# archinetai/audio-diffusion-pytorch

Measured on AMD Instinct MI355X. Metric: denoising steps/s (UNetV0 fwd+bwd) at [B,2,2**18], higher is better.
Workload: dtype f32; 1 GPU; BASELINE.json configs[1]: unconditional DiffusionModel(UNetV0 channels=[8,32,64,128,256,512,512,1024,1024], factors=[1,4,4,4,2,2,2,2,2], items=[1,2,2,2,2,2,2,4,4]) fwd+bwd, audio=randn(4,2,2**18) per GPU, random-init weights; per_gpu_batch=4, global_batch=4, length=262144, launch=hipGraph replay, parallelism=single, collective_world_size=1, collectives_in_graph=False, optimizer=none (the metric is fwd+bwd; gradients for all 176M parameters are produced)

## Files before the change

### audio_diffusion_pytorch_amd/_C.py

```python
import ctypes
import os
from ctypes import POINTER, Structure, c_float, c_int, c_int64, c_void_p

import torch

_PKG_DIR = os.path.dirname(os.path.abspath(__file__))
LIB_PATH = os.path.join(_PKG_DIR, "libadp_hip.so")

_lib = None
_allow_cpu = False

ERRORS = {-1: "bad shape", -2: "unsupported configuration", -3: "misaligned pointer", -4: "kernel launch failed",
          -5: "null pointer"}

P = c_void_p
I = c_int64
F = c_float


class ConvDesc(Structure):
    _fields_ = [(n, c_void_p) for n in ("x", "x2", "w", "bias", "pro_stats", "pro_gamma", "pro_beta", "e_scale",
                                        "res", "out", "out_pre")] + \
               [(n, c_int64) for n in ("B", "R", "R1", "Lin", "M", "N", "KT", "stride", "dil", "pad", "up",
                                       "transposed", "prologue", "groups", "store", "sp", "e_bstride")] + \
# ... 99 lines not shown
    "adp_arv_step": (c_int, [P, P, P, I, I, I, I, P, P, P]),
    "adp_arv_plane": (c_int, [P, I, I, I, P, P]),
}

ABI["adp_lt.h"] = {
    "adp_lt_conv_out_len": (I, [I, I, I, I]),
    "adp_lt_convt_out_len": (I, [I, I, I, I]),
    "adp_lt_conv": (c_int, [P, P, I, I, I, I, I, I, I, I, P, P]),
    "adp_lt_convt": (c_int, [P, P, I, I, I, I, I, I, I, I, I, P, P]),
    "adp_lt_wgrad_ws_bytes": (I, [I, I, I, I, I]),
    "adp_lt_wgrad": (c_int, [P, P, I, I, I, I, I, I, I, I, I, P, P, P]),
}

ABI["adp_enc.h"] = {
    "adp_enc_down_out_len": (I, [I, I]),
    "adp_enc_down_fwd": (c_int, [P, P, P, I, I, I, I, I, P, P]),
    "adp_enc_down_dgrad": (c_int, [P, P, I, I, I, I, I, P, P]),
    "adp_enc_down_wgrad_ws_bytes": (I, [I, I, I, I, I]),
    "adp_enc_down_wgrad": (c_int, [P, P, I, I, I, I, I, P, P, P, P]),
    "adp_enc_tanh_fwd": (c_int, [P, I, P, P]),
    "adp_enc_tanh_bwd": (c_int, [P, P, I, P, P]),
}

ABI["adp_t5.h"] = {
    "adp_t5_embed": (c_int, [P, P, I, I, I, P, P]),
    "adp_t5_rmsnorm": (c_int, [P, P, I, I, F, P, P]),
    "adp_t5_linear_ws_bytes": (I, [I, I, I]),
    "adp_t5_linear": (c_int, [P, P, P, I, I, I, I, P, P, P]),
    "adp_t5_attn": (c_int, [P, P, P, P, I, I, I, I, I, P, P]),
}

ABI["adp_rng.h"] = {
    "adp_philox_bits": (c_int, [P, I, P, P]),
    "adp_randn": (c_int, [P, I, P, P]),
    "adp_v_inpaint_step_rng": (c_int, [P, P, P, P, P, P, I, P, P]),
}

ABI["adp_clip.h"] = {
    "adp_clip_ws_bytes": (I, [I, I]),
    "adp_clip_scale": (c_int, [P, P, P, I, I, I, F, F, P, P, P]),
    "adp_clip_apply": (c_int, [P, P, I, I, P, P]),
    "adp_clip_step": (c_int, [P, P, P, P, P, I, P, I, I, P, P, P, P]),
}

ABI["adp_gated.h"] = {
    "adp_gated_linear_ws_bytes": (I, [I, I, I]),
    "adp_gated_linear": (c_int, [P, P, P, I, I, I, I, P, P, P]),
}

ABI["adp_sde.h"] = {
    "adp_v_step_eta": (c_int, [P, P, P, P, I, P, I, I, P, P]),
}

ABI["adp_rf.h"] = {
    "adp_rf_noise": (c_int, [P, P, P, I, I, P, P, P]),
    "adp_rf_step": (c_int, [P, P, P, P, I, I, P, I, I, P, P, P]),
}

ABI["adp_edm.h"] = {
    "adp_edm_noise": (c_int, [P, P, P, F, I, I, P, P, P]),
    "adp_edm_step": (c_int, [P, P, P, P, P, I, I, P, I, I, P, P, P]),
}

ABI["adp_repaint.h"] = {
    "adp_repaint_v_step": (c_int, [P, P, P, P, P, P, I, P, I, I, P, P]),
    "adp_repaint_rf_step": (c_int, [P, P, P, P, P, P, I, P, I, I, P, P]),
    "adp_repaint_k_step": (c_int, [P, P, P, P, P, P, I, P, I, I, P, P]),
}

ABI["adp_spec.h"] = {
    "adp_spec_loss_ws_bytes": (I, [I, I, I, I, P, P, I]),
    "adp_spec_loss_fwd": (c_int, [P, P, I, I, I, I, P, P, P, P, F, F, F, F, F, F, P, P, P]),
    "adp_spec_loss_bwd": (c_int, [P, P, P, P, I, I, I, I, P, P, P, P, P, F, F, F, F, F, F, P, P, P]),
    "adp_spec_fir": (c_int, [P, P, I, I, I, P, P]),
}

ABI["adp_distill.h"] = {
    "adp_distill_comb": (c_int, [P, P, P, P, I, I, I, P, P]),
    "adp_distill_wmse_ws_bytes": (I, [I, I]),
    "adp_distill_wmse_fwd": (c_int, [P, P, P, I, I, P, P, P]),
    "adp_distill_wmse_bwd": (c_int, [P, P, P, P, I, I, P, P]),
}


HEADER_SOURCE = {"adp_ar.h": "elementwise.hip", "adp_lt.h": "lt.hip", "adp_enc.h": "encoder.hip", "adp_t5.h": "t5.hip",
                 "adp_rng.h": "rng.hip", "adp_clip.h": "clip.hip", "adp_gated.h": "gated.hip", "adp_sde.h": "sde.hip",
                 "adp_rf.h": "rf.hip", "adp_edm.h": "edm.hip", "adp_repaint.h": "repaint.hip", "adp_spec.h": "spectral.hip",
                 "adp_distill.h": "distill.hip"}

SIGNATURES = {}
for _header, _table in ABI.items():
    for _name in _table:
        if _name in SIGNATURES:
            _first = next(h for h, t in ABI.items() if _name in t)
            raise ImportError(f"{_name} is in the tables of both {_first} and {_header}: one header declares an entry point")
    SIGNATURES.update(_table)


def _bind(path: str):
    lib = ctypes.CDLL(path)
    for name, (res, args) in SIGNATURES.items():
        fn = getattr(lib, name)
        fn.restype = res
        fn.argtypes = args
    return lib


def lib():
    global _lib
    if _lib is None:
        if not os.path.exists(LIB_PATH):
            raise RuntimeError(
                f"{LIB_PATH} is missing: build the gfx950 kernels first "
                "(python -m audio_diffusion_pytorch_amd.build or __graft_entry__.build()); "
                "audio_diffusion_pytorch_amd has no CPU/PyTorch fallback path")
        _lib = _bind(LIB_PATH)
    return _lib


def _testing_use_library(path, allow_cpu: bool):
    global _lib, _allow_cpu
    _lib = _bind(path) if path is not None else None
    _allow_cpu = allow_cpu


def stream() -> int:
    if _allow_cpu and not torch.cuda.is_available():
        return 0
    return torch.cuda.current_stream().cuda_stream


def ptr(t, dtype=torch.float32):
    if t is None:
        return None
    if t.dtype != dtype:
        raise TypeError(f"adp kernel argument must be {dtype}; got {t.dtype}")
    if not t.is_contiguous():
        raise ValueError("adp kernels need contiguous tensors")
    if not t.is_cuda and not _allow_cpu:
        raise RuntimeError("adp kernels run on MI355X (HIP) tensors only; got a CPU tensor and there is no CPU path")
    return t.data_ptr()


def check(code: int, what: str):
    if code != 0:
        raise RuntimeError(f"{what} failed: {ERRORS.get(code, code)} ({code})")


PROFILE = None
_TAG = None
REPLAY = None


def tag(**meta):
    global _TAG
    if PROFILE is not None:
        _TAG = meta


def _decode_trace(text: str) -> str:
    import re
    names = []
    for item in text.split("\n"):
        if not item:
            continue
        kern, _, site = item.partition("@")
        kern = kern.strip()
        while kern.startswith("(") and kern.endswith(")"):
            kern = kern[1:-1].strip()
        m = re.search(r"\[(?:with )?([^\]]*)\]\s*$", site)
        env = {}
# ... 60 lines not shown
```

### audio_diffusion_pytorch_amd/csrc/linear.hip

```cpp
#include "adp_rt.h"
#include "adp.h"
#include "conv_internal.h"

namespace {

constexpr int LIN_BMAX = 16;
constexpr int LIN_KC = 1024;
constexpr int LIN_RPW = 8;
static inline int64_t lin_rpw(int64_t N) { return N >= 4096 ? LIN_RPW : 1; }

__device__ __forceinline__ float lin_act(float x, int act) {
  return act == 1 ? adp_silu(x) : (act == 2 ? adp_gelu(x) : x);
}

__device__ __forceinline__ void lin_stage(const float* x, int64_t B, int64_t K, int64_t k0, int kc, int act,
                                          float* xs) {
  for (int e = threadIdx.x; e < (int)B * LIN_KC; e += 256) {
    const int b = e / LIN_KC, k = e - b * LIN_KC;
    xs[e] = (k < kc) ? lin_act(x[b * K + k0 + k], act) : 0.0f;
  }
}

template <int BT>
__global__ __launch_bounds__(256) void linear_fwd_kernel(const float* x, const float* w, const float* bias,
                                                         int64_t B, int64_t K, int64_t N, int act, int post,
                                                         int64_t ybstride, float* y, int rpw) {
  __shared__ float xs[BT * LIN_KC];
  const int lane = threadIdx.x & 63, wave = threadIdx.x >> 6;
  const int64_t nbase = ((int64_t)blockIdx.x * 4 + wave) * rpw;
  const bool vec = (K % 4 == 0);
  for (int64_t k0 = 0; k0 < K; k0 += LIN_KC) {
    const int kc = (int)((K - k0) < LIN_KC ? (K - k0) : LIN_KC);
    __syncthreads();
    lin_stage(x, B, K, k0, kc, act, xs);
    __syncthreads();
    for (int r = 0; r < rpw; ++r) {
      const int64_t n = nbase + r;
      if (n >= N) break;
      float acc[BT];
#pragma unroll
      for (int b = 0; b < BT; ++b) acc[b] = 0.0f;
      const float* wr = w + n * K + k0;
#pragma unroll 4
      for (int k = lane * 4; k < kc; k += 256) {
        float w0, w1, w2, w3;
        if (vec) {
          const float4 wv = *reinterpret_cast<const float4*>(wr + k);
          w0 = wv.x; w1 = wv.y; w2 = wv.z; w3 = wv.w;
        } else {
          w0 = wr[k];
          w1 = (k + 1 < kc) ? wr[k + 1] : 0.0f;
          w2 = (k + 2 < kc) ? wr[k + 2] : 0.0f;
          w3 = (k + 3 < kc) ? wr[k + 3] : 0.0f;
        }
#pragma unroll
        for (int b = 0; b < BT; ++b) {
          if (b < B) {
            const float* xr = xs + b * LIN_KC + k;
            acc[b] = fmaf(w0, xr[0], fmaf(w1, xr[1], fmaf(w2, xr[2], fmaf(w3, xr[3], acc[b]))));
          }
        }
      }
#pragma unroll
      for (int b = 0; b < BT; ++b) {
        const float sres = adp_wave_sum(acc[b]);
        if (lane == 0 && b < B) {
          float v = sres + ((k0 == 0 && bias) ? bias[n] : 0.0f);
          if (k0 > 0) v += y[b * ybstride + n];
          if (post == 2 && k0 + LIN_KC >= K) v = adp_gelu(v);
          y[b * ybstride + n] = v;
        }
      }
    }
  }
}

constexpr int LIN_NR = 64;

template <int BT>
__global__ __launch_bounds__(256) void linear_bwd_data_kernel(const float* dy, int64_t dybstride, const float* w,
                                                              int64_t B, int64_t K, int64_t N, float* ws) {
  constexpr int NR = LIN_NR, RPW = NR / 4;
  __shared__ float dys[BT * NR];
  __shared__ __attribute__((aligned(16))) float part[3][BT][256];
// ... 38 lines not shown
    }
  }
  if (wave > 0) {
#pragma unroll
    for (int b = 0; b < BT; ++b)
#pragma unroll
      for (int q = 0; q < 4; ++q) part[wave - 1][b][lane * 4 + q] = acc[b][q];
  }
  __syncthreads();
  if (wave == 0 && k < K) {
#pragma unroll
    for (int b = 0; b < BT; ++b) {
      if (b < B) {
        float* o = ws + ((int64_t)blockIdx.x * B + b) * K + k;
#pragma unroll
        for (int q = 0; q < 4; ++q) {
          const float v = ((acc[b][q] + part[0][b][lane * 4 + q]) + part[1][b][lane * 4 + q]) + part[2][b][lane * 4 + q];
          if (k + q < K) o[q] = v;
        }
      }
    }
  }
}

template <int BT>
__global__ __launch_bounds__(256) void linear_bwd_weight_kernel(const float* dy, int64_t dybstride, const float* x,
                                                                int64_t B, int64_t K, int64_t N, int act,
                                                                int accumulate, float* dw, float* dbias, int rpw) {
  __shared__ __attribute__((aligned(16))) float xs[BT * LIN_KC];
  const int lane = threadIdx.x & 63, wave = threadIdx.x >> 6;
  const int64_t nbase = ((int64_t)blockIdx.x * 4 + wave) * rpw;
  const bool vec = (K % 4 == 0) && ((reinterpret_cast<uintptr_t>(dw) & 15) == 0);
  float dfirst[BT];
#pragma unroll
  for (int b = 0; b < BT; ++b) dfirst[b] = (b < B && nbase < N) ? dy[b * dybstride + nbase] : 0.0f;
  for (int64_t k0 = 0; k0 < K; k0 += LIN_KC) {
    const int kc = (int)((K - k0) < LIN_KC ? (K - k0) : LIN_KC);
    __syncthreads();
    lin_stage(x, B, K, k0, kc, act, xs);
    __syncthreads();
    for (int r = 0; r < rpw; ++r) {
      const int64_t n = nbase + r;
      if (n >= N) break;
      float d[BT];
#pragma unroll
      for (int b = 0; b < BT; ++b) d[b] = r == 0 ? dfirst[b] : ((b < B) ? dy[b * dybstride + n] : 0.0f);
      if (k0 == 0 && dbias && lane == 0) {
        float s = 0.0f;
#pragma unroll
        for (int b = 0; b < BT; ++b) s += d[b];
        dbias[n] = accumulate ? dbias[n] + s : s;
      }
      float* orow = dw + n * K + k0;
      if (vec) {
        for (int k = lane * 4; k < kc; k += 256) {
          f32x4 sv = {0.0f, 0.0f, 0.0f, 0.0f};
#pragma unroll
          for (int b = 0; b < BT; ++b)
            if (b < B) {
              const f32x4 xv = *reinterpret_cast<const f32x4*>(xs + b * LIN_KC + k);
#pragma unroll
              for (int j = 0; j < 4; ++j) sv[j] = fmaf(d[b], xv[j], sv[j]);
            }
          if (accumulate) {
            const f32x4 o = *reinterpret_cast<const f32x4*>(orow + k);
#pragma unroll
            for (int j = 0; j < 4; ++j) sv[j] += o[j];
          }
          *reinterpret_cast<f32x4*>(orow + k) = sv;
        }
      } else {
        for (int k = lane; k < kc; k += 64) {
          float s = 0.0f;
#pragma unroll
          for (int b = 0; b < BT; ++b)
            if (b < B) s = fmaf(d[b], xs[b * LIN_KC + k], s);
          orow[k] = accumulate ? orow[k] + s : s;
        }
      }
    }
  }
}

}

#define LIN_DISPATCH(B, CALL)                   \
  do {                                          \
    if ((B) <= 4) { constexpr int BT = 4; CALL; }        \
    else if ((B) <= 8) { constexpr int BT = 8; CALL; }   \
    else { constexpr int BT = 16; CALL; }       \
  } while (0)

extern "C" int adp_linear_fwd(const float* x, const float* w, const float* bias, int64_t B, int64_t K, int64_t N,
                              int64_t act, int64_t post, float* y, int64_t y_bstride, void* stream) {
  if (!x || !w || !y) return ADP_ERR_NULL;
  if (B <= 0 || B > LIN_BMAX || K <= 0 || N <= 0) return ADP_ERR_SHAPE;
  if (act < 0 || act > 2 || (post != 0 && post != 2)) return ADP_ERR_UNSUPPORTED;
  if (y_bstride == 0) y_bstride = N;
  const int64_t rpw = lin_rpw(N);
  dim3 grid((unsigned)adp_cdiv(N, 4 * rpw));
  LIN_DISPATCH(B, ADP_LAUNCH((linear_fwd_kernel<BT>), grid, dim3(256), stream, x, w, bias, B, K, N, (int)act,
                             (int)post, y_bstride, y, (int)rpw));
  return ADP_LAUNCH_OK();
}

extern "C" int64_t adp_linear_bwd_data_ws_bytes(int64_t B, int64_t K, int64_t N) {
  if (B <= 0 || K <= 0 || N <= 0) return ADP_ERR_SHAPE;
  return adp_cdiv(N, LIN_NR) * B * K * (int64_t)sizeof(float);
}

extern "C" int adp_linear_bwd_data(const float* dy, int64_t dy_bstride, const float* w, int64_t B, int64_t K,
                                   int64_t N, int64_t accumulate, float* dxa, float* ws, void* stream) {
  if (!dy || !w || !dxa || !ws) return ADP_ERR_NULL;
  if (B <= 0 || B > LIN_BMAX || K <= 0 || N <= 0) return ADP_ERR_SHAPE;
  if (dy_bstride == 0) dy_bstride = N;
  const int64_t P = adp_cdiv(N, LIN_NR);
  if (P > 2147483647 || adp_cdiv(K, 256) > 65535) return ADP_ERR_SHAPE;
  LIN_DISPATCH(B, ADP_LAUNCH((linear_bwd_data_kernel<BT>), dim3((unsigned)P, (unsigned)adp_cdiv(K, 256)), dim3(256),
                             stream, dy, dy_bstride, w, B, K, N, ws));
  return adp_wgrad_reduce(ws, P, B * K, 0, dxa, nullptr, (int)accumulate, stream);
}

extern "C" int adp_linear_bwd_weight(const float* dy, int64_t dy_bstride, const float* x, int64_t B, int64_t K,
                                     int64_t N, int64_t act, int64_t accumulate, float* dw, float* dbias,
                                     void* stream) {
  if (!dy || !x || !dw) return ADP_ERR_NULL;
  if (B <= 0 || B > LIN_BMAX || K <= 0 || N <= 0) return ADP_ERR_SHAPE;
  if (act < 0 || act > 2) return ADP_ERR_UNSUPPORTED;
  if (dy_bstride == 0) dy_bstride = N;
  const int64_t rpw = lin_rpw(N);
  dim3 grid((unsigned)adp_cdiv(N, 4 * rpw));
  LIN_DISPATCH(B, ADP_LAUNCH((linear_bwd_weight_kernel<BT>), grid, dim3(256), stream, dy, dy_bstride, x, B, K, N,
                             (int)act, (int)accumulate, dw, dbias, (int)rpw));
  return ADP_LAUNCH_OK();
}
```

### audio_diffusion_pytorch_amd/ops.py

```python
import contextlib
import ctypes
import math
import os
from ctypes import byref
from typing import Optional, Tuple

import torch
from torch import Tensor

from . import _C
from ._C import ConvDesc, WgradDesc, ptr

GN_EPS = 1e-5
MODULATION_LN_EPS = 1e-5
ATTENTION_LN_EPS = 1e-5


def _ws(nbytes: int, like: Tensor) -> Tensor:
    return torch.empty(max(1, (nbytes + 3) // 4), dtype=torch.float32, device=like.device)


def conv_out_len(Lin: int, KT: int, stride: int, dil: int, pad: int, up: int) -> int:
    return (Lin * up + 2 * pad - dil * (KT - 1) - 1) // stride + 1

# ... 377 lines not shown
    return dx, dgb


LIN_ROWS = 16


def linear_fwd(x: Tensor, w: Tensor, bias: Optional[Tensor], act: int = 0, post: int = 0,
               y: Optional[Tensor] = None) -> Tensor:
    B, K = x.shape
    N = w.shape[0]
    if y is None:
        y = torch.empty((B, N), dtype=torch.float32, device=x.device)
    _C.tag(bytes=4 * (w.numel() + x.numel() + y.numel()), shape=f"B{B} K{K} N{N}")
    for b0 in range(0, B, LIN_ROWS):
        nb = min(LIN_ROWS, B - b0)
        _C.call("adp_linear_fwd", ptr(x[b0:b0 + nb]), ptr(w), ptr(bias), nb, K, N, act, post, ptr(y[b0:b0 + nb]), N,
                _C.stream())
    return y


def linear_bwd_data(dy: Tensor, w: Tensor, dxa: Optional[Tensor] = None, accumulate: bool = False) -> Tensor:
    B, N = dy.shape
    K = w.shape[1]
    if dxa is None:
        dxa = torch.empty((B, K), dtype=torch.float32, device=dy.device)
    ws = _ws(_C.query("adp_linear_bwd_data_ws_bytes", min(B, LIN_ROWS), K, N), dy)
    _C.tag(bytes=4 * (w.numel() + B * N + dxa.numel()), shape=f"B{B} K{K} N{N}")
    for b0 in range(0, B, LIN_ROWS):
        nb = min(LIN_ROWS, B - b0)
        _C.call("adp_linear_bwd_data", ptr(dy[b0:b0 + nb]), N, ptr(w), nb, K, N, int(accumulate),
                ptr(dxa[b0:b0 + nb]), ptr(ws), _C.stream())
    return dxa


def linear_bwd_weight(dy: Tensor, x: Tensor, act: int = 0, dw: Optional[Tensor] = None,
                      dbias: Optional[Tensor] = None, want_bias: bool = True, accumulate: bool = False,
                      rows: Optional[int] = None, dy_bstride: Optional[int] = None):
    if rows is None:
        B, N = dy.shape
        dy_bstride = N
        dy = dy.reshape(-1)
    else:
        B, N = x.shape[0], rows
    K = x.shape[1]
    if dw is None:
        dw = torch.empty((N, K), dtype=torch.float32, device=dy.device)
    if dbias is None and want_bias:
        dbias = torch.empty((N,), dtype=torch.float32, device=dy.device)
    _C.tag(bytes=4 * (dw.numel() + B * N + x.numel()), shape=f"B{B} K{K} N{N}")
    for b0 in range(0, B, LIN_ROWS):
        nb = min(LIN_ROWS, B - b0)
        _C.call("adp_linear_bwd_weight", ptr(dy[b0 * dy_bstride:]), dy_bstride, ptr(x[b0:b0 + nb]), nb, K, N, act,
                int(accumulate or b0 > 0), ptr(dw), ptr(dbias), _C.stream())
    return dw, dbias


def time_fourier_fwd(t: Tensor, w: Tensor) -> Tensor:
    B, H = t.shape[0], w.shape[0]
    four = torch.empty((B, 2 * H + 1), dtype=torch.float32, device=t.device)
    _C.call("adp_time_fourier_fwd", ptr(t), ptr(w), B, H, ptr(four), _C.stream())
    return four


def time_fourier_bwd(t: Tensor, w: Tensor, dfour: Tensor, dw: Optional[Tensor] = None,
                     accumulate: bool = False) -> Tensor:
    B, H = t.shape[0], w.shape[0]
    if dw is None:
        dw = torch.empty_like(w)
    _C.call("adp_time_fourier_bwd", ptr(t), ptr(w), ptr(dfour), B, H, int(accumulate), ptr(dw), _C.stream())
    return dw


def act_fwd(x: Tensor, act: int) -> Tensor:
    y = torch.empty_like(x)
    _C.call("adp_act_fwd", ptr(x), x.numel(), act, ptr(y), _C.stream())
    return y


def act_bwd(x: Tensor, dy: Tensor, act: int, dx: Optional[Tensor] = None, accumulate: bool = False) -> Tensor:
    if dx is None:
        dx = torch.empty_like(x)
    _C.call("adp_act_bwd", ptr(x), ptr(dy), x.numel(), act, int(accumulate), ptr(dx), _C.stream())
    return dx


def skipmod_bwd(g: Tensor, x: Tensor, scale: Tensor, scale_bstride: int, dscale: Tensor, dscale_bstride: int,
                dx: Optional[Tensor] = None) -> Tensor:
    B, C, L = x.shape
    if dx is None:
        dx = torch.empty_like(x)
    ws = _ws(_C.query("adp_skipmod_bwd_ws_bytes", B, C, L), x)
    _C.tag(bytes=12 * x.numel(), shape=f"B{B} C{C} L{L}")
    _C.call("adp_skipmod_bwd", ptr(g), ptr(x), ptr(scale), scale_bstride, B, C, L, ptr(dx), ptr(dscale),
            dscale_bstride, ptr(ws), _C.stream())
    return dx


def v_noise(x: Tensor, noise: Tensor, sigma: Tensor):
    B = x.shape[0]
    per = x.numel() // B
    x_noisy, v_target = torch.empty_like(x), torch.empty_like(x)
    _C.call("adp_v_noise", ptr(x), ptr(noise), ptr(sigma), B, per, ptr(x_noisy), ptr(v_target), _C.stream())
    return x_noisy, v_target


def mse_fwd(v_pred: Tensor, v_target: Tensor) -> Tensor:
    n = v_pred.numel()
    loss = torch.empty((), dtype=torch.float32, device=v_pred.device)
    ws = _ws(_C.query("adp_mse_ws_bytes", n), v_pred)
    _C.call("adp_mse_fwd", ptr(v_pred), ptr(v_target), n, ptr(loss), ptr(ws), _C.stream())
    return loss


def mse_bwd(v_pred: Tensor, v_target: Tensor, gloss: Optional[Tensor]) -> Tensor:
    dv = torch.empty_like(v_pred)
    _C.call("adp_mse_bwd", ptr(v_pred), ptr(v_target), ptr(gloss), v_pred.numel(), ptr(dv), _C.stream())
    return dv


def _stft_res(res) -> ctypes.Array:
    flat = [int(v) for triple in res for v in triple]
    return (ctypes.c_int64 * len(flat))(*flat)


def stft_loss_fwd(x: Tensor, y: Tensor, res, w_sc: float, w_log: float, w_lin: float, eps: float):
    L = x.shape[-1]
    rows, arr = x.numel() // L, _stft_res(res)
    loss = torch.empty((), dtype=torch.float32, device=x.device)
    ws = _ws(_C.query("adp_stft_loss_ws_bytes", rows, L, len(res), arr, 0), x)
    _C.call("adp_stft_loss_fwd", ptr(x), ptr(y), rows, L, len(res), arr, w_sc, w_log, w_lin, eps, ptr(loss), ptr(ws),
            _C.stream())
    return loss, ws


def stft_loss_bwd(x: Tensor, y: Tensor, gloss: Optional[Tensor], ws_fwd: Tensor, res, w_sc: float, w_log: float,
                  w_lin: float, eps: float) -> Tensor:
    L = x.shape[-1]
    rows, arr = x.numel() // L, _stft_res(res)
    dx = torch.empty_like(x)
    ws = _ws(_C.query("adp_stft_loss_ws_bytes", rows, L, len(res), arr, 1), x)
    _C.call("adp_stft_loss_bwd", ptr(x), ptr(y), ptr(gloss), ptr(ws_fwd), rows, L, len(res), arr, w_sc, w_log, w_lin, eps,
            ptr(dx), ptr(ws), _C.stream())
    return dx


def _spec_bins(res, n_bins) -> ctypes.Array:
    return (ctypes.c_int64 * len(res))(*([0] * len(res) if n_bins is None else [int(v) for v in n_bins]))


def spec_loss_fwd(x: Tensor, y: Tensor, pair: bool, res, n_bins, fb: Optional[Tensor], mel_range: Optional[Tensor],
                  w_sc: float, w_log: float, w_lin: float, eps: float, w_sum: float = 1.0, w_diff: float = 1.0):
    L = x.shape[-1]
    rows, arr, bins = x.numel() // L, _stft_res(res), _spec_bins(res, n_bins)
    loss = torch.empty((), dtype=torch.float32, device=x.device)
    ws = _ws(_C.query("adp_spec_loss_ws_bytes", rows, L, int(pair), len(res), arr, bins, 0), x)
    _C.call("adp_spec_loss_fwd", ptr(x), ptr(y), rows, L, int(pair), len(res), arr, bins, ptr(fb),
            ptr(mel_range, torch.int32), w_sc, w_log, w_lin, eps, w_sum, w_diff, ptr(loss), ptr(ws), _C.stream())
    return loss, ws


def spec_loss_bwd(x: Tensor, y: Tensor, gloss: Optional[Tensor], ws_fwd: Tensor, pair: bool, res, n_bins,
                  fb: Optional[Tensor], mel_range: Optional[Tensor], bin_range: Optional[Tensor], w_sc: float, w_log: float,
                  w_lin: float, eps: float, w_sum: float = 1.0, w_diff: float = 1.0) -> Tensor:
    L = x.shape[-1]
    rows, arr, bins = x.numel() // L, _stft_res(res), _spec_bins(res, n_bins)
    dx = torch.empty_like(x)
# ... 930 lines not shown
```

### audio_diffusion_pytorch_amd/unet.py

```python
from typing import Dict, List, Optional, Sequence

import os

import torch
import torch.nn as nn
from torch import Tensor

from . import ops
from .attention import PendingLN

ITEM_RESNET = "resnet"
ITEM_MODULATION = "modulation"
ITEM_INJECT = "inject"
ITEM_ATTENTION = "attention"
ITEM_CROSS_ATTENTION = "cross_attention"

TIME_EMBED_DIM = 256
TIME_NUM_LAYERS = 2
ACT_NONE, ACT_SILU, ACT_GELU = 0, 1, 2

A_UNET_SEMANTICS = {
    "DOWNSAMPLE_WIDTH": 1,
    "UPSAMPLE_KERNEL_SIZE": 3,
    "RESNET_KERNEL_SIZE": 3,
# ... 335 lines not shown
                embedding: Optional[Tensor] = None, channels: Optional[Sequence[Optional[Tensor]]] = None,
                x_append: Optional[Tensor] = None, conditioning: Optional[Tensor] = None) -> Tensor:
        if conditioning is not None:
            if torch.is_grad_enabled() and (x.requires_grad or any(p.requires_grad for _, p in self._named_params())):
                raise RuntimeError("UNetV0.forward(conditioning=...) is an inference-only path (torch.no_grad())")
            assert features is None and conditioning.shape == (x.shape[0], self.bank_total), \
                "conditioning: [B, bank_total] rows of conditioning_table, without `features`"
        if self.use_time:
            assert time is not None, "TimeConditioningPlugin requires time in forward"
        elif time is not None:
            raise TypeError("UNetV0(use_time_conditioning=False).forward() takes 1 positional argument (x); "
                            "`time` was given")
        if self.bank_total > 0 and not self.use_time:
            assert features is not None, "ModulationItem requires `features` when use_time_conditioning=False"
        params = [p for _, p in self._named_params()]
        ctx_list = [c for c in (channels or []) if c is not None]
        grad_on = torch.is_grad_enabled()
        if not x.is_cuda:
            return _UNetFn.apply(self, x, time, features, embedding, x_append, channels, len(ctx_list), conditioning,
                                 grad_on, *ctx_list, *params)
        for t in (time, features, embedding, x_append, conditioning, *ctx_list, params[0]):
            if t is not None and t.device != x.device:
                raise RuntimeError(f"UNetV0: every tensor must live on the input's device {x.device}; got {t.device}")
        with torch.cuda.device(x.device):
            return _UNetFn.apply(self, x, time, features, embedding, x_append, channels, len(ctx_list), conditioning,
                                 grad_on, *ctx_list, *params)

    @torch.no_grad()
    def conditioning_table(self, times: Tensor) -> Optional[Tensor]:
        if not (self.use_time and self.bank_total > 0):
            return None
        run = _Run(self, False)
        return run.conditioning(times.reshape(-1), None)


NATIVE_FACTORS = (1, 2, 4)
SKIP_CAT_SCALE = 2 ** -0.5
POISON_GRADS = os.environ.get("ADP_DEBUG_POISON", "0") == "1"
GN_EPILOGUE = int(os.environ.get("ADP_GN_EPILOGUE", "1"))


def _grad_buffer(shape, device) -> Tensor:
    buf = torch.empty(shape, dtype=torch.float32, device=device)
    if POISON_GRADS:
        buf.fill_(float("nan"))
    return buf


MOD_LN_FUSE = os.environ.get("ADP_MOD_LN_FUSE", "1") != "0"

MOD_LN_BWD_FUSE = os.environ.get("ADP_MOD_LN_BWD_FUSE", "1") != "0"

ACT_MATERIALIZE_MIN_C = int(os.environ.get("ADP_ACT_MATERIALIZE_MIN_C", "64"))


class _Run:

    def __init__(self, net: UNetV0Net, need_grad: bool):
        self.net = net
        self.need_grad = need_grad
        self.tape: List = []
        self.grads: Dict[str, Tensor] = {}
        net._named_params()
        self.pnames = net._pname_cache
        self.gn: Optional[ops.GnPart] = None
        self.ln_ready = None
        self.mod_sums = ops.ModulationSums()
        self.wpark = ops.WgradPark() if os.environ.get("ADP_WGRAD_PARK", "1") != "0" else None

    def g(self, p: nn.Parameter) -> Tensor:
        try:
            return self.grads[self.pnames[id(p)]]
        except KeyError:
            raise RuntimeError("UNetV0: a parameter the kernels read is not one of the net's registered Parameters (replaced "
                               "between forward and backward, or wrapped by nn.utils.parametrize -- not supported by the "
                               "one-node U-Net: its gradient would have no slot in the flat gradient buffer)") from None

    def gspan(self, p_first: nn.Parameter, numel: int) -> Tensor:
        a, _ = self.net._param_offsets()[self.pnames[id(p_first)]]
        return self.flat[a:a + numel]

    def conditioning(self, time: Tensor, features: Optional[Tensor], ss_pre: Optional[Tensor] = None):
        n = self.net
        self.ss_all = self.dss_all = None
        if ss_pre is not None:
            assert not self.need_grad
            self.feats = None
            self.ss_all = ss_pre.contiguous()
            return self.ss_all
        if n.use_time:
            t = time.reshape(-1).to(torch.float32).contiguous()
            four = ops.time_fourier_fwd(t, n.time_weights)
            pre = [ops.linear_fwd(four, n.time_linear.weight, n.time_linear.bias)]
            acts = [ops.act_fwd(pre[0], ACT_GELU)]
            for lin in n.time_mlp:
                pre.append(ops.linear_fwd(acts[-1], lin.weight, lin.bias))
                acts.append(ops.act_fwd(pre[-1], ACT_GELU))
            feats = acts[-1] if features is None else ops.add(features.contiguous(), acts[-1])
            self.t, self.four, self.pre, self.acts = t, four, pre, acts
        else:
            feats = features.contiguous() if features is not None else None
        self.feats = feats
        if n.bank_total > 0:
            self.ss_all = ops.linear_fwd(feats, n.bank_weight, n.bank_bias, act=ACT_SILU)
            if self.need_grad:
                self.dss_all = _grad_buffer(self.ss_all.shape, self.ss_all.device)
        return self.ss_all

    def conditioning_backward(self) -> Tensor:
        n = self.net
        if n.bank_total == 0:
            return None
        assert not self.mod_sums.items, "dss_all is read while second stages of Modulation backwards are still parked"
        dfa = ops.linear_bwd_data(self.dss_all, n.bank_weight)
        dfeat = ops.act_bwd(self.feats, dfa, ACT_SILU)
        if not n.use_time:
            return dfeat
        dcur = dfeat
        lins = [n.time_linear] + list(n.time_mlp)
        for i in range(len(lins) - 1, -1, -1):
            dp = ops.act_bwd(self.pre[i], dcur, ACT_GELU)
            xin = self.four if i == 0 else self.acts[i - 1]
            ops.linear_bwd_weight(dp, xin, act=ACT_NONE, dw=self.g(lins[i].weight), dbias=self.g(lins[i].bias))
            dcur = ops.linear_bwd_data(dp, lins[i].weight)
        ops.time_fourier_bwd(self.t, n.time_weights, dcur, dw=self.g(n.time_weights))
        return dfeat

    def bank_grad_all(self) -> None:
        n = self.net
        if n.bank_total > 0:
            assert not self.mod_sums.items, "parked Modulation sums while the bank's gradient is formed"
            ops.linear_bwd_weight(self.dss_all.view(-1), self.feats, act=ACT_SILU, dw=self.g(n.bank_weight),
                                  dbias=self.g(n.bank_bias), rows=n.bank_total, dy_bstride=n.bank_total)

    def bank_grad_for_depth(self, d: int, defer: bool = False):
        n = self.net
        a, b = n.bank_depth_rows[d] if n.bank_total > 0 else (0, 0)
        self.mod_sums.flush(a, b)
        assert not any(a <= it[0] < b for it in self.mod_sums.items), "parked Modulation sums inside the rows being read"
        if b > a and not defer:
            K = n.mf
            ops.linear_bwd_weight(self.dss_all.view(-1)[a:], self.feats, act=ACT_SILU,
                                  dw=self.g(n.bank_weight)[a:b], dbias=self.g(n.bank_bias)[a:b], rows=b - a,
                                  dy_bstride=n.bank_total)
        return a, b

    def ss(self, key):
        off, nout = self.net.bank_slices[key]
        return self.ss_all.view(-1)[off:], (self.dss_all.view(-1)[off:] if self.need_grad else None)

    def gn_part_for(self, C: int) -> Optional[ops.GnPart]:
        if GN_EPILOGUE and (C // self.net.groups) % 4 == 0:
            return ops.GnPart()
        return None

    def gn_stats_of(self, x: Tensor) -> Tensor:
        G = self.net.groups
        if self.gn is not None and self.gn.covers(x):
            return ops.gn_finalize(self.gn.part, G)
        return ops.gn_stats(x, G)

    def gn_stats_act_of(self, x: Tensor, gnp):
        G = self.net.groups
        if self.gn is not None and self.gn.covers(x):
            part = self.gn.part
            if (x.shape[1] // G // 4) * part.shape[2] <= 1024:
                return ops.gn_finalize_act(x, part, G, gnp.weight, gnp.bias)
            st = ops.gn_finalize(part, G)
            return st, ops.gn_act(x, st, G, gnp.weight, gnp.bias)
        return ops.gn_stats_act(x, G, gnp.weight, gnp.bias)

    def resnet(self, p, x: Tensor) -> Tensor:
        G = self.net.groups
        if x.shape[1] >= ACT_MATERIALIZE_MIN_C and x.shape[0] * x.shape[1] <= 65535:
            return self.resnet_wide(p, x)
        st1 = self.gn_stats_of(x)
        self.gn = self.gn_part_for(x.shape[1])
        h1 = ops.conv1d(x, p.conv1.weight, p.conv1.bias, pad=1, prologue=1, pro_stats=st1, pro_gamma=p.gn1.weight,
                        pro_beta=p.gn1.bias, groups=G, gn=self.gn)
        st2 = self.gn_stats_of(h1)
        self.gn = None
        y = ops.conv1d(h1, p.conv2.weight, p.conv2.bias, pad=1, prologue=1, pro_stats=st2, pro_gamma=p.gn2.weight,
                       pro_beta=p.gn2.bias, groups=G, res=x)
        if self.need_grad:
            def bwd(gy):
                ops.conv1d_wgrad(h1, gy, 3, pad=1, park=self.wpark, prologue=1, pro_stats=st2, pro_gamma=p.gn2.weight,
                                 pro_beta=p.gn2.bias, groups=G, dw=self.g(p.conv2.weight), dbias=self.g(p.conv2.bias))
                gb2 = ops.GnBwdPart(h1, st2, p.gn2.weight, p.gn2.bias, G)
                dact2 = ops.conv1d(gy, p.conv2.weight, None, pad=1, transposed=True, gnb=gb2)
                dh1, _, _ = ops.gn_silu_bwd(h1, dact2, st2, p.gn2.weight, p.gn2.bias, G, dgamma=self.g(p.gn2.weight),
                                            dbeta=self.g(p.gn2.bias), ab=gb2.ab)
                ops.conv1d_wgrad(x, dh1, 3, pad=1, park=self.wpark, prologue=1, pro_stats=st1, pro_gamma=p.gn1.weight,
                                 pro_beta=p.gn1.bias, groups=G, dw=self.g(p.conv1.weight), dbias=self.g(p.conv1.bias))
                gb1 = ops.GnBwdPart(x, st1, p.gn1.weight, p.gn1.bias, G)
                dact1 = ops.conv1d(dh1, p.conv1.weight, None, pad=1, transposed=True, gnb=gb1)
                dx, _, _ = ops.gn_silu_bwd(x, dact1, st1, p.gn1.weight, p.gn1.bias, G, dres=gy,
                                           dgamma=self.g(p.gn1.weight), dbeta=self.g(p.gn1.bias), ab=gb1.ab)
                return dx
            self.tape.append((bwd, None))
        return y

    def resnet_wide(self, p, x: Tensor) -> Tensor:
        G = self.net.groups
        st1, a1 = self.gn_stats_act_of(x, p.gn1)
        self.gn = self.gn_part_for(x.shape[1])
        h1 = ops.conv1d(a1, p.conv1.weight, p.conv1.bias, pad=1, gn=self.gn)
        st2, a2 = self.gn_stats_act_of(h1, p.gn2)
        self.gn = None
# ... 184 lines not shown
    @staticmethod
    def forward(ctx, net: UNetV0Net, x, time, features, embedding, x_append, channels, n_ctx, cond_pre, grad_on, *rest):
        ctx_list, params = rest[:n_ctx], rest[n_ctx:]
        need_grad = bool(grad_on) and any(ctx.needs_input_grad)
        run = _Run(net, need_grad)
        run.skip_grads = []
        run.ctx_index = {}
        j = 0
        for d, c in enumerate(channels or []):
            if c is not None:
                run.ctx_index[d] = j
                j += 1
        run.ctx_grads = [None] * n_ctx if need_grad else None
        run.ctx_needs = [bool(c.requires_grad) for c in ctx_list]
        x = x.contiguous()
        x2 = x_append.contiguous() if x_append is not None else None
        run.conditioning(time, features, cond_pre if not need_grad else None)
        run.emb_grad = None
        run.want_emb_grad = bool(embedding is not None and ctx.needs_input_grad[4])
        run.want_x2_grad = bool(need_grad and x2 is not None and ctx.needs_input_grad[5])
        run.x2_grad = None
        run.ctx_bank = None
        if embedding is not None and os.environ.get("ADP_CTX_BANK", "1") != "0":
            from .attention import CtxBank
            run.ctx_bank = CtxBank.prepare(run, embedding.contiguous())
            if run.ctx_bank is not None:
                net._ctx_bank_runs = getattr(net, "_ctx_bank_runs", 0) + 1
        y = run.block(0, x, x2, embedding.contiguous() if embedding is not None else None, channels,
                      need_dx=bool(ctx.needs_input_grad[1]))
        ctx.run = run
        ctx.params = params
        ctx.n_ctx = n_ctx
        ctx.has_features = features is not None
        ctx.has_embedding = embedding is not None
        return y

    @staticmethod
    def backward(ctx, gy):
        run: _Run = ctx.run
        if run is None:
            raise RuntimeError("the U-Net tape was released by a previous backward through this forward; "
                               "run the forward again (retain_graph is not supported by the one-node U-Net)")
        net = run.net
        named = net._named_params()
        offs = net._param_offsets()
        total = max(b for _, b in offs.values())
        flat = _grad_buffer((total,), gy.device)
        run.flat = flat
        views = []
        for name, p in named:
            a, b = offs[name]
            v = flat[a:b].view(p.shape)
            run.grads[name] = v
            views.append(v)
        hook = getattr(net, "_grad_ready_hook", None)
        defer_bank = hook is None and os.environ.get("ADP_BANK_DEFER", "1") != "0"
        ctx_depth = net.ctx_final_depth()
        g = gy.contiguous()
        for fn, tag in reversed(run.tape):
            g = fn(g)
            if tag is not None:
                if run.wpark is not None:
                    run.wpark.flush()
                ra, rb = run.bank_grad_for_depth(tag, defer=defer_bank)
                if hook is not None:
                    if run.wpark is not None:
                        run.wpark.join()
                    hook(flat, *net.block_param_range(tag))
                    if rb > ra:
                        w0 = offs["bank_weight"][0]
                        hook(flat, w0 + ra * net.mf, w0 + rb * net.mf)
                if tag == ctx_depth:
                    if run.ctx_bank is not None:
                        run.ctx_bank.backward(run)
                        if hook is not None:
                            net._ctx_bank_hooked_backwards = getattr(net, "_ctx_bank_hooked_backwards", 0) + 1
                    if hook is not None:
                        ca, cb = net.ctx_param_range()
                        if cb > ca:
                            hook(flat, ca, cb)
        run.mod_sums.flush()
        if run.wpark is not None:
            run.wpark.flush()
        if defer_bank:
            run.bank_grad_all()
        dfeat = run.conditioning_backward()
        if run.wpark is not None:
            run.wpark.join()
        if hook is not None:
            for a, b in net.nonblock_param_ranges():
                hook(flat, a, b)
            hook(flat, None, None)
        gx = g if ctx.needs_input_grad[1] else None
        gfeat = dfeat if (ctx.has_features and ctx.needs_input_grad[3]) else None
        gemb = None
        if ctx.has_embedding and ctx.needs_input_grad[4] and run.emb_grad is not None:
            gemb = run.emb_grad.transpose(1, 2)
        gctx = tuple(run.ctx_grads) if run.ctx_grads is not None else (None,) * ctx.n_ctx
        run.grads.clear()
        run.flat = None
        ctx.run = None
        gx2 = run.x2_grad
        run.x2_grad = None
        out = (None, gx, None, gfeat, gemb, gx2, None, None, None, None) + gctx + tuple(views)
        del views, flat, v
        return out
```

Measured before the change: 89.42 denoising steps/s.

## Fuse conditioning MLP linear, activation, and weight/data gradients into combined kernels

Adds conditioning-specific linear kernels. The forward pass writes the pre-activation and the GELU output in one launch. The backward pass computes the data gradient and the weight/bias gradients in a single pass over the weight matrix, and the split-K reduction applies the activation derivatives. This replaces separate linear_fwd/act_fwd and linear_bwd_data/act_bwd/linear_bwd_weight launches for the time MLP and the modulation bank, cutting launches and repeated reads of the large bank weight. The path is on by default through an environment switch and adds a workspace plus a second reduction kernel per call.

Measured after the change: 88.92 denoising steps/s. About the same (-0.6%).

```diff
diff --git a/audio_diffusion_pytorch_amd/_C.py b/audio_diffusion_pytorch_amd/_C.py
--- a/audio_diffusion_pytorch_amd/_C.py
+++ b/audio_diffusion_pytorch_amd/_C.py
@@ -205,11 +205,17 @@
     "adp_distill_wmse_bwd": (c_int, [P, P, P, P, I, I, P, P]),
 }
 
+ABI["adp_cond.h"] = {
+    "adp_cond_linear_fwd": (c_int, [P, P, P, I, I, I, I, I, P, P, I, P]),
+    "adp_cond_linear_bwd": (c_int, [P, I, P, P, I, I, I, I, I, P, P, P, P]),
+    "adp_cond_reduce_act": (c_int, [P, I, I, P, I, P, P, I, P, P]),
+}
+
 
 HEADER_SOURCE = {"adp_ar.h": "elementwise.hip", "adp_lt.h": "lt.hip", "adp_enc.h": "encoder.hip", "adp_t5.h": "t5.hip",
                  "adp_rng.h": "rng.hip", "adp_clip.h": "clip.hip", "adp_gated.h": "gated.hip", "adp_sde.h": "sde.hip",
                  "adp_rf.h": "rf.hip", "adp_edm.h": "edm.hip", "adp_repaint.h": "repaint.hip", "adp_spec.h": "spectral.hip",
-                 "adp_distill.h": "distill.hip"}
+                 "adp_distill.h": "distill.hip", "adp_cond.h": "linear.hip"}
 
 SIGNATURES = {}
 for _header, _table in ABI.items():
diff --git a/audio_diffusion_pytorch_amd/csrc/linear.hip b/audio_diffusion_pytorch_amd/csrc/linear.hip
--- a/audio_diffusion_pytorch_amd/csrc/linear.hip
+++ b/audio_diffusion_pytorch_amd/csrc/linear.hip
@@ -1,5 +1,6 @@
 #include "adp_rt.h"
 #include "adp.h"
+#include "adp_cond.h"
 #include "conv_internal.h"
 
 namespace {
@@ -204,6 +205,220 @@
   }
 }
 
+__device__ __forceinline__ float lin_dact(float x, int act) {
+  return act == 1 ? adp_dsilu(x) : (act == 2 ? adp_dgelu(x) : 1.0f);
+}
+
+template <int BT>
+__global__ __launch_bounds__(256) void cond_linear_fwd_kernel(const float* x, const float* w, const float* bias, int64_t B,
+                                                              int64_t K, int64_t N, int act, int post, int64_t ybstride,
+                                                              float* y, float* pre, int rpw) {
+  __shared__ float xs[BT * LIN_KC];
+  const int lane = threadIdx.x & 63, wave = threadIdx.x >> 6;
+  const int64_t nbase = ((int64_t)blockIdx.x * 4 + wave) * rpw;
+  const bool vec = (K % 4 == 0);
+  for (int64_t k0 = 0; k0 < K; k0 += LIN_KC) {
+    const int kc = (int)((K - k0) < LIN_KC ? (K - k0) : LIN_KC);
+    __syncthreads();
+    lin_stage(x, B, K, k0, kc, act, xs);
+    __syncthreads();
+    for (int r = 0; r < rpw; ++r) {
+      const int64_t n = nbase + r;
+      if (n >= N) break;
+      float acc[BT];
+#pragma unroll
+      for (int b = 0; b < BT; ++b) acc[b] = 0.0f;
+      const float* wr = w + n * K + k0;
+#pragma unroll 4
+      for (int k = lane * 4; k < kc; k += 256) {
+        float w0, w1, w2, w3;
+        if (vec) {
+          const float4 wv = *reinterpret_cast<const float4*>(wr + k);
+          w0 = wv.x; w1 = wv.y; w2 = wv.z; w3 = wv.w;
+        } else {
+          w0 = wr[k];
+          w1 = (k + 1 < kc) ? wr[k + 1] : 0.0f;
+          w2 = (k + 2 < kc) ? wr[k + 2] : 0.0f;
+          w3 = (k + 3 < kc) ? wr[k + 3] : 0.0f;
+        }
+#pragma unroll
+        for (int b = 0; b < BT; ++b) {
+          if (b < B) {
+            const float* xr = xs + b * LIN_KC + k;
+            acc[b] = fmaf(w0, xr[0], fmaf(w1, xr[1], fmaf(w2, xr[2], fmaf(w3, xr[3], acc[b]))));
+          }
+        }
+      }
+      const bool last = k0 + LIN_KC >= K;
+#pragma unroll
+      for (int b = 0; b < BT; ++b) {
+        const float sres = adp_wave_sum(acc[b]);
+        if (lane == 0 && b < B) {
+          float v = sres + ((k0 == 0 && bias) ? bias[n] : 0.0f);
+          if (k0 > 0) v += y[b * ybstride + n];
+          if (last && pre) pre[b * ybstride + n] = v;
+          if (post == 2 && last) v = adp_gelu(v);
+          y[b * ybstride + n] = v;
+        }
+      }
+    }
+  }
+}
+
+template <int BT>
+__global__ __launch_bounds__(256) void cond_linear_bwd_kernel(const float* __restrict__ dy, int64_t dybstride,
+                                                              const float* __restrict__ w, const float* __restrict__ x,
+                                                              int64_t B, int64_t K, int64_t N, int act, int accumulate,
+                                                              float* __restrict__ dw, float* __restrict__ dbias,
+                                                              float* __restrict__ ws) {
+  constexpr int NR = LIN_NR, RPW = NR / 4;
+  __shared__ float dys[BT * NR];
+  __shared__ __attribute__((aligned(16))) float part[3][BT][256];
+  const int lane = threadIdx.x & 63, wave = threadIdx.x >> 6;
+  const int64_t n0 = (int64_t)blockIdx.x * NR;
+  const int nr = (int)((N - n0) < NR ? (N - n0) : NR);
+  const int64_t k = (int64_t)blockIdx.y * 256 + lane * 4;
+  const bool vec = (K % 4 == 0);
+  const bool wvec = vec && ((reinterpret_cast<uintptr_t>(dw) & 15) == 0);
+  float xa[BT][4];
+#pragma unroll
+  for (int b = 0; b < BT; ++b)
+#pragma unroll
+    for (int q = 0; q < 4; ++q) xa[b][q] = (dw && b < B && k + q < K) ? lin_act(x[b * K + k + q], act) : 0.0f;
+  for (int e = threadIdx.x; e < BT * NR; e += 256) {
+    const int b = e / NR, j = e - b * NR;
+    dys[e] = (b < B && j < nr) ? dy[b * dybstride + n0 + j] : 0.0f;
+  }
+  __syncthreads();
+  float acc[BT][4];
+#pragma unroll
+  for (int b = 0; b < BT; ++b) acc[b][0] = acc[b][1] = acc[b][2] = acc[b][3] = 0.0f;
+  if (k < K) {
+#pragma unroll 8
+    for (int jj = 0; jj < RPW; ++jj) {
+      const int j = wave * RPW + jj;
+      if (j < nr) {
+        const float* wr = w + (n0 + j) * K + k;
+        float w0, w1, w2, w3;
+        if (vec) {
+          const float4 wv = *reinterpret_cast<const float4*>(wr);
+          w0 = wv.x; w1 = wv.y; w2 = wv.z; w3 = wv.w;
+        } else {
+          w0 = wr[0];
+          w1 = (k + 1 < K) ? wr[1] : 0.0f;
+          w2 = (k + 2 < K) ? wr[2] : 0.0f;
+          w3 = (k + 3 < K) ? wr[3] : 0.0f;
+        }
+        float d[BT];
+#pragma unroll
+        for (int b = 0; b < BT; ++b) {
+          d[b] = dys[b * NR + j];
+          acc[b][0] = fmaf(d[b], w0, acc[b][0]);
+          acc[b][1] = fmaf(d[b], w1, acc[b][1]);
+          acc[b][2] = fmaf(d[b], w2, acc[b][2]);
+          acc[b][3] = fmaf(d[b], w3, acc[b][3]);
+        }
+        if (dw) {
+          if (dbias && blockIdx.y == 0 && lane == 0) {
+            float s = 0.0f;
+#pragma unroll
+            for (int b = 0; b < BT; ++b) s += d[b];
+            dbias[n0 + j] = accumulate ? dbias[n0 + j] + s : s;
+          }
+          f32x4 sv = {0.0f, 0.0f, 0.0f, 0.0f};
+#pragma unroll
+          for (int b = 0; b < BT; ++b)
+            if (b < B) {
+#pragma unroll
+              for (int q = 0; q < 4; ++q) sv[q] = fmaf(d[b], xa[b][q], sv[q]);
+            }
+          float* orow = dw + (n0 + j) * K + k;
+          if (wvec) {
+            if (accumulate) {
+              const f32x4 o = *reinterpret_cast<const f32x4*>(orow);
+#pragma unroll
+              for (int q = 0; q < 4; ++q) sv[q] += o[q];
+            }
+            *reinterpret_cast<f32x4*>(orow) = sv;
+          } else {
+#pragma unroll
+            for (int q = 0; q < 4; ++q)
+              if (k + q < K) orow[q] = accumulate ? orow[q] + sv[q] : sv[q];
+          }
+        }
+      }
+    }
+  }
+  if (wave > 0) {
+#pragma unroll
+    for (int b = 0; b < BT; ++b)
+#pragma unroll
+      for (int q = 0; q < 4; ++q) part[wave - 1][b][lane * 4 + q] = acc[b][q];
+  }
+  __syncthreads();
+  if (wave == 0 && k < K) {
+#pragma unroll
+    for (int b = 0; b < BT; ++b) {
+      if (b < B) {
+        float* o = ws + ((int64_t)blockIdx.x * B + b) * K + k;
+#pragma unroll
+        for (int q = 0; q < 4; ++q) {
+          const float v = ((acc[b][q] + part[0][b][lane * 4 + q]) + part[1][b][lane * 4 + q]) + part[2][b][lane * 4 + q];
+          if (k + q < K) o[q] = v;
+        }
+      }
+    }
+  }
+}
+
+__device__ __forceinline__ void cond_reduce_out(float sum, int64_t i, const float* pre1, int act1, float* out1,
+                                                const float* pre2, int act2, float* out2) {
+  const float v1 = act1 ? sum * lin_dact(pre1[i], act1) : sum;
+  out1[i] = v1;
+  if (out2) out2[i] = v1 * lin_dact(pre2[i], act2);
+}
+
+__global__ __launch_bounds__(1024) void cond_reduce_act_kernel(const float* ws, int64_t nsplit, int64_t cnt,
+                                                               const float* pre1, int act1, float* out1,
+                                                               const float* pre2, int act2, float* out2) {
+  __shared__ float part[16][64];
+  const int il = threadIdx.x & 63, ks = threadIdx.x >> 6;
+  const int64_t i = (int64_t)blockIdx.x * 64 + il;
+  float s = 0.0f;
+  if (i < cnt) {
+    const float* col = ws + i;
+    int64_t k = ks;
+    for (; k + 7 * 16 < nsplit; k += 8 * 16) {
+      float v[8];
+#pragma unroll
+      for (int u = 0; u < 8; ++u) v[u] = col[(k + 16 * u) * cnt];
+#pragma unroll
+      for (int u = 0; u < 8; ++u) s += v[u];
+    }
+    for (; k < nsplit; k += 16) s += col[k * cnt];
+  }
+  part[ks][il] = s;
+  __syncthreads();
+  if (ks == 0 && i < cnt) {
+    float sum = 0.0f;
+#pragma unroll
+    for (int k = 0; k < 16; ++k) sum += part[k][il];
+    cond_reduce_out(sum, i, pre1, act1, out1, pre2, act2, out2);
+  }
+}
+
+__global__ __launch_bounds__(256) void cond_reduce_act_small_kernel(const float* ws, int64_t nsplit, int64_t cnt,
+                                                                    const float* pre1, int act1, float* out1,
+                                                                    const float* pre2, int act2, float* out2) {
+  const int64_t i = (int64_t)blockIdx.x * 256 + threadIdx.x;
+  if (i < cnt) {
+    float s = 0.0f;
+#pragma unroll 8
+    for (int64_t k = 0; k < nsplit; ++k) s += ws[k * cnt + i];
+    cond_reduce_out(s, i, pre1, act1, out1, pre2, act2, out2);
+  }
+}
+
 }
 
 #define LIN_DISPATCH(B, CALL)                   \
@@ -256,3 +471,45 @@
                              (int)act, (int)accumulate, dw, dbias, (int)rpw));
   return ADP_LAUNCH_OK();
 }
+
+extern "C" int adp_cond_linear_fwd(const float* x, const float* w, const float* bias, int64_t B, int64_t K, int64_t N,
+                                   int64_t act, int64_t post, float* y, float* pre, int64_t y_bstride, void* stream) {
+  if (!x || !w || !y) return ADP_ERR_NULL;
+  if (B <= 0 || B > LIN_BMAX || K <= 0 || N <= 0) return ADP_ERR_SHAPE;
+  if (act < 0 || act > 2 || (post != 0 && post != 2)) return ADP_ERR_UNSUPPORTED;
+  if (y_bstride == 0) y_bstride = N;
+  const int64_t rpw = lin_rpw(N);
+  dim3 grid((unsigned)adp_cdiv(N, 4 * rpw));
+  LIN_DISPATCH(B, ADP_LAUNCH((cond_linear_fwd_kernel<BT>), grid, dim3(256), stream, x, w, bias, B, K, N, (int)act,
+                             (int)post, y_bstride, y, pre, (int)rpw));
+  return ADP_LAUNCH_OK();
+}
+
+extern "C" int adp_cond_linear_bwd(const float* dy, int64_t dy_bstride, const float* w, const float* x, int64_t B,
+                                   int64_t K, int64_t N, int64_t act, int64_t accumulate, float* dw, float* dbias,
+                                   float* ws, void* stream) {
+  if (!dy || !w || !ws || (dw && !x) || (dbias && !dw)) return ADP_ERR_NULL;
+  if (B <= 0 || B > LIN_BMAX || K <= 0 || N <= 0) return ADP_ERR_SHAPE;
+  const int64_t P = adp_cdiv(N, LIN_NR);
+  if (P > 2147483647 || adp_cdiv(K, 256) > 65535) return ADP_ERR_SHAPE;
+  if (dw && (act < 0 || act > 2)) return ADP_ERR_UNSUPPORTED;
+  if (dy_bstride == 0) dy_bstride = N;
+  LIN_DISPATCH(B, ADP_LAUNCH((cond_linear_bwd_kernel<BT>), dim3((unsigned)P, (unsigned)adp_cdiv(K, 256)), dim3(256),
+                             stream, dy, dy_bstride, w, x, B, K, N, (int)act, (int)(accumulate & 1), dw, dbias, ws));
+  return ADP_LAUNCH_OK();
+}
+
+extern "C" int adp_cond_reduce_act(const float* ws, int64_t P, int64_t n, const float* pre1, int64_t act1, float* out1,
+                                   const float* pre2, int64_t act2, float* out2, void* stream) {
+  if (!ws || !out1 || (act1 != 0 && !pre1) || (out2 && !pre2)) return ADP_ERR_NULL;
+  if (P <= 0 || n <= 0 || adp_cdiv(n, 64) > 2147483647) return ADP_ERR_SHAPE;
+  if (act1 < 0 || act1 > 2 || act2 < 0 || act2 > 2) return ADP_ERR_UNSUPPORTED;
+  if (P <= 8) {
+    ADP_LAUNCH(cond_reduce_act_small_kernel, dim3((unsigned)adp_cdiv(n, 256)), dim3(256), stream, ws, P, n, pre1, (int)act1,
+               out1, pre2, (int)act2, out2);
+    return ADP_LAUNCH_OK();
+  }
+  ADP_LAUNCH(cond_reduce_act_kernel, dim3((unsigned)adp_cdiv(n, 64)), dim3(1024), stream, ws, P, n, pre1, (int)act1, out1,
+             pre2, (int)act2, out2);
+  return ADP_LAUNCH_OK();
+}
diff --git a/audio_diffusion_pytorch_amd/ops.py b/audio_diffusion_pytorch_amd/ops.py
--- a/audio_diffusion_pytorch_amd/ops.py
+++ b/audio_diffusion_pytorch_amd/ops.py
@@ -483,6 +483,52 @@
         dx = torch.empty_like(x)
     _C.call("adp_act_bwd", ptr(x), ptr(dy), x.numel(), act, int(accumulate), ptr(dx), _C.stream())
     return dx
+
+
+def cond_fused() -> bool:
+    return os.environ.get("ADP_COND_FUSED", "1") != "0"
+
+
+def cond_linear_fwd(x: Tensor, w: Tensor, bias: Optional[Tensor], act: int = 0, post: int = 0, want_pre: bool = False):
+    B, K = x.shape
+    N = w.shape[0]
+    y = torch.empty((B, N), dtype=torch.float32, device=x.device)
+    pre = torch.empty_like(y) if want_pre else None
+    _C.tag(bytes=4 * (w.numel() + x.numel() + y.numel() * (2 if want_pre else 1)), shape=f"B{B} K{K} N{N}")
+    for b0 in range(0, B, LIN_ROWS):
+        nb = min(LIN_ROWS, B - b0)
+        _C.call("adp_cond_linear_fwd", ptr(x[b0:b0 + nb]), ptr(w), ptr(bias), nb, K, N, act, post, ptr(y[b0:b0 + nb]),
+                ptr(pre[b0:b0 + nb]) if want_pre else None, N, _C.stream())
+    return y, pre
+
+
+def cond_linear_bwd(dy: Tensor, w: Tensor, x: Tensor, act: int = 0, dw: Optional[Tensor] = None,
+                    dbias: Optional[Tensor] = None, rows: Optional[int] = None, dy_bstride: Optional[int] = None,
+                    d1=None, d2=None):
+    B, K = x.shape
+    if rows is None:
+        N = dy.shape[1]
+        dy_bstride = N
+        dy = dy.reshape(-1)
+    else:
+        N = rows
+    nb_max = min(B, LIN_ROWS)
+    ws = _ws(_C.query("adp_linear_bwd_data_ws_bytes", nb_max, K, N), x)
+    P = (N + 63) // 64
+    out1 = torch.empty((B, K), dtype=torch.float32, device=x.device)
+    out2 = torch.empty_like(out1) if d2 is not None else None
+    pre1, act1 = d1 if d1 is not None else (None, 0)
+    pre2, act2 = d2 if d2 is not None else (None, 0)
+    for b0 in range(0, B, LIN_ROWS):
+        nb = min(LIN_ROWS, B - b0)
+        _C.tag(bytes=4 * (w.numel() * (2 if dw is not None else 1) + nb * N + nb * K * (P + 1)), shape=f"B{nb} K{K} N{N}")
+        _C.call("adp_cond_linear_bwd", ptr(dy[b0 * dy_bstride:]), dy_bstride, ptr(w), ptr(x[b0:b0 + nb]), nb, K, N, act,
+                int(b0 > 0), ptr(dw), ptr(dbias), ptr(ws), _C.stream())
+        _C.tag(bytes=4 * nb * K * (P + 1 + (d1 is not None) + 2 * (d2 is not None)), shape=f"P{P} n{nb * K}")
+        _C.call("adp_cond_reduce_act", ptr(ws), P, nb * K, ptr(pre1[b0:b0 + nb]) if pre1 is not None else None, act1,
+                ptr(out1[b0:b0 + nb]), ptr(pre2[b0:b0 + nb]) if pre2 is not None else None, act2,
+                ptr(out2[b0:b0 + nb]) if out2 is not None else None, _C.stream())
+    return out1, out2
 
 
 def skipmod_bwd(g: Tensor, x: Tensor, scale: Tensor, scale_bstride: int, dscale: Tensor, dscale_bstride: int,
diff --git a/audio_diffusion_pytorch_amd/unet.py b/audio_diffusion_pytorch_amd/unet.py
--- a/audio_diffusion_pytorch_amd/unet.py
+++ b/audio_diffusion_pytorch_amd/unet.py
@@ -441,6 +441,7 @@
 
     def conditioning(self, time: Tensor, features: Optional[Tensor], ss_pre: Optional[Tensor] = None):
         n = self.net
+        fused = ops.cond_fused()
         self.ss_all = self.dss_all = None
         if ss_pre is not None:
             assert not self.need_grad
@@ -450,27 +451,39 @@
         if n.use_time:
             t = time.reshape(-1).to(torch.float32).contiguous()
             four = ops.time_fourier_fwd(t, n.time_weights)
-            pre = [ops.linear_fwd(four, n.time_linear.weight, n.time_linear.bias)]
-            acts = [ops.act_fwd(pre[0], ACT_GELU)]
-            for lin in n.time_mlp:
-                pre.append(ops.linear_fwd(acts[-1], lin.weight, lin.bias))
-                acts.append(ops.act_fwd(pre[-1], ACT_GELU))
+            pre, acts = [], []
+            for lin in [n.time_linear] + list(n.time_mlp):
+                xin = four if not acts else acts[-1]
+                if fused:
+                    a, p = ops.cond_linear_fwd(xin, lin.weight, lin.bias, post=ACT_GELU, want_pre=True)
+                else:
+                    p = ops.linear_fwd(xin, lin.weight, lin.bias)
+                    a = ops.act_fwd(p, ACT_GELU)
+                pre.append(p)
+                acts.append(a)
             feats = acts[-1] if features is None else ops.add(features.contiguous(), acts[-1])
             self.t, self.four, self.pre, self.acts = t, four, pre, acts
         else:
             feats = features.contiguous() if features is not None else None
         self.feats = feats
         if n.bank_total > 0:
-            self.ss_all = ops.linear_fwd(feats, n.bank_weight, n.bank_bias, act=ACT_SILU)
+            if fused:
+                self.ss_all, _ = ops.cond_linear_fwd(feats, n.bank_weight, n.bank_bias, act=ACT_SILU)
+            else:
+                self.ss_all = ops.linear_fwd(feats, n.bank_weight, n.bank_bias, act=ACT_SILU)
             if self.need_grad:
                 self.dss_all = _grad_buffer(self.ss_all.shape, self.ss_all.device)
         return self.ss_all
 
-    def conditioning_backward(self) -> Tensor:
+    def conditioning_backward(self, bank_grad: bool = False) -> Tensor:
         n = self.net
         if n.bank_total == 0:
             return None
         assert not self.mod_sums.items, "dss_all is read while second stages of Modulation backwards are still parked"
+        if ops.cond_fused():
+            return self._conditioning_backward_fused(bank_grad)
+        if bank_grad:
+            self.bank_grad_all()
         dfa = ops.linear_bwd_data(self.dss_all, n.bank_weight)
         dfeat = ops.act_bwd(self.feats, dfa, ACT_SILU)
         if not n.use_time:
@@ -483,6 +496,22 @@
             ops.linear_bwd_weight(dp, xin, act=ACT_NONE, dw=self.g(lins[i].weight), dbias=self.g(lins[i].bias))
             dcur = ops.linear_bwd_data(dp, lins[i].weight)
         ops.time_fourier_bwd(self.t, n.time_weights, dcur, dw=self.g(n.time_weights))
+        return dfeat
+
+    def _conditioning_backward_fused(self, bank_grad: bool) -> Tensor:
+        n = self.net
+        dw, db = (self.g(n.bank_weight), self.g(n.bank_bias)) if bank_grad else (None, None)
+        last = (self.pre[-1], ACT_GELU) if n.use_time else None
+        dfeat, dp = ops.cond_linear_bwd(self.dss_all.view(-1), n.bank_weight, self.feats, act=ACT_SILU, dw=dw, dbias=db,
+                                        rows=n.bank_total, dy_bstride=n.bank_total, d1=(self.feats, ACT_SILU), d2=last)
+        if not n.use_time:
+            return dfeat
+        lins = [n.time_linear] + list(n.time_mlp)
+        for i in range(len(lins) - 1, -1, -1):
+            xin = self.four if i == 0 else self.acts[i - 1]
+            dp, _ = ops.cond_linear_bwd(dp, lins[i].weight, xin, act=ACT_NONE, dw=self.g(lins[i].weight),
+                                        dbias=self.g(lins[i].bias), d1=(self.pre[i - 1], ACT_GELU) if i > 0 else None)
+        ops.time_fourier_bwd(self.t, n.time_weights, dp, dw=self.g(n.time_weights))
         return dfeat
 
     def bank_grad_all(self) -> None:
@@ -833,9 +862,7 @@
         run.mod_sums.flush()
         if run.wpark is not None:
             run.wpark.flush()
-        if defer_bank:
-            run.bank_grad_all()
-        dfeat = run.conditioning_backward()
+        dfeat = run.conditioning_backward(bank_grad=defer_bank)
         if run.wpark is not None:
             run.wpark.join()
         if hook is not None:
diff --git a/include/adp_cond.h b/include/adp_cond.h
--- /dev/null
+++ b/include/adp_cond.h
@@ -0,0 +1,21 @@
+#ifndef ADP_COND_H
+#define ADP_COND_H
+#include "adp.h"
+
+#ifdef __cplusplus
+extern "C" {
+#endif
+
+int adp_cond_linear_fwd(const float* x, const float* w, const float* bias, int64_t B, int64_t K, int64_t N, int64_t act,
+                        int64_t post, float* y, float* pre, int64_t y_bstride, void* stream);
+
+int adp_cond_linear_bwd(const float* dy, int64_t dy_bstride, const float* w, const float* x, int64_t B, int64_t K,
+                        int64_t N, int64_t act, int64_t accumulate, float* dw, float* dbias, float* ws, void* stream);
+
+int adp_cond_reduce_act(const float* ws, int64_t P, int64_t n, const float* pre1, int64_t act1, float* out1,
+                        const float* pre2, int64_t act2, float* out2, void* stream);
+
+#ifdef __cplusplus
+}
+#endif
+#endif
```
